# plurigrid/moose

Measured on AMD Instinct MI355X. Metric: replicated fixed(14,23) matmul elems/sec, higher is better.
Workload: dtype fixed(14,23) over Z_2^128 (exact multi-modular int8-MFMA GEMM)

## Files before the change

### csrc/gemm_crt.hip

```cpp
#include <hip/hip_runtime.h>

#include <algorithm>
#include <cmath>
#include <cstdint>
#include <cstdlib>
#include <cstring>
#include <mutex>

#include "hip_attr.h"
#include "moosex.h"

void mx_ws_note(int dev, int64_t want, bool ok);
bool mx_ws_malloc(void** p, int64_t bytes);
void mx_ws_shared_note(void);

namespace {

using u64 = uint64_t;
using u128 = unsigned __int128;
typedef int v4i __attribute__((ext_vector_type(4)));
typedef int v16i __attribute__((ext_vector_type(16)));

constexpr int kMaxMod = 48;
constexpr int kModuli[kMaxMod] = {256, 253, 251, 249, 247, 241, 239, 235, 233, 229, 227, 223,
                                  217, 211, 199, 197, 193, 191, 181, 179, 173, 167, 163, 157,
// ... 279 lines not shown
    emit(ob + boff);
    if (src.n > 0 && src.dual[b]) {
#pragma unroll
      for (int j = 0; j < 16; ++j) {
        const int64_t k = k0 + j;
        if (row < R && k < K) {
          T e = 0;
#pragma unroll
          for (int w = 0; w < NW; ++w) e |= (T)v[j][w] << (32 * w);
          e += TRANS ? x1[k * R + row] : x1[row * K + k];
#pragma unroll
          for (int w = 0; w < NW; ++w) v[j][w] = (uint32_t)(e >> (32 * w));
        }
      }
      emit(ob + src.dual[b] + boff);
    }
  }
}

template <class T>
__global__ void __launch_bounds__(256)
    k_add_pair(const T* __restrict__ a, const T* __restrict__ b, T* __restrict__ o, int64_t n) {
  for (int64_t i = blockIdx.x * (int64_t)blockDim.x + threadIdx.x; i < n;
       i += (int64_t)gridDim.x * blockDim.x)
    o[i] = a[i] + b[i];
}

__device__ inline int64_t xcd_remap(int64_t bid, int64_t nwg) {
  const int64_t q = nwg / 8, r = nwg % 8;
  const int64_t x = bid % 8;
// ... 691 lines not shown
      hipLaunchKernelGGL((k_crt_prep<T, true, 128, false>), grid, dim3(256), 0, st, X0, X1, R, K,
                         xs, mode, out, tiles, nkb, nkb_s, tb.pb, src);
    return;
  }
  if (!is_b)
    hipLaunchKernelGGL((k_crt_prep<T, false, BM>), grid, dim3(256), 0, st, X0, X1, R, K, xs, mode,
                       out, tiles, nkb, nkb_s, tb.pa, src);
  else if (rows == 256)
    hipLaunchKernelGGL((k_crt_prep<T, true, 256>), grid, dim3(256), 0, st, X0, X1, R, K, xs, mode,
                       out, tiles, nkb, nkb_s, tb.pb, src);
  else
    hipLaunchKernelGGL((k_crt_prep<T, true, 128>), grid, dim3(256), 0, st, X0, X1, R, K, xs, mode,
                       out, tiles, nkb, nkb_s, tb.pb, src);
}

int dma_mask() {
  const char* e = std::getenv("MOOSEX_CRT_DMA_MASK");
  return e ? std::atoi(e) : 3;
}

template <int WR, int WC, int BN, int MINW, bool M16, int STG = kStages, int IL = 0>
void launch_variant(const CPlan& p, const Tables& tb, int64_t batch, const int8_t* ra,
                    const int8_t* rb, int8_t* cr, int bcast, int roll, hipStream_t st,
                    int amap = 0, int bmap = 0) {
  constexpr int lds = STG * (kImg + BN * BK);
  const void* fn = M16 ? (const void*)k_crt_gemm16<WR, WC, BN, MINW, STG, IL>
                       : (const void*)k_crt_gemm<WR, WC, BN, MINW>;
  ensure_lds_attr(fn, lds, st);
  const dim3 grid((unsigned)(p.tiles_m * p.tiles_n), (unsigned)(batch * p.n));
  if constexpr (M16)
// ... 127 lines not shown
    rb = rbw;
  }
  if (roll)
    launch_prep<T>(p, tb, false, batch, M, K, a_bstride, A0, A0, 0, ra, st, p.a_nkb);
  else
    launch_prep<T>(p, tb, false, a_bc ? 1 : batch, M, K, a_bstride, A0, A1, mode, ra, st);
  launch_crt_gemm(p, tb, batch, ra, rb, cr, (a_bc ? 1 : 0) | (b_bc ? 2 : 0),
                  (int)(((roll % batch) + batch) % batch), st);
  launch_recon<T>(p, tb, batch, M, N, cr, C, accumulate, st);
  const hipError_t e = hipGetLastError();
  return e != hipSuccess ? -100 - (int)e : 0;
}

template <class T>
int run_crt_asym(int64_t M, int64_t N, int64_t K, const T* S0, const T* S1, const T* T0,
                 const T* T1, int rolled, T* C, hipStream_t st) {
  constexpr int words = sizeof(T) / 8;
  if (K % BK || !crt_mfma16()) return -7;
  if (2 * K > (1 << 15)) return -6;
  const CPlan p = make_cplan(words, 3, M, N, K, 1, true);
  if (p.n < 0) return -6;
  const Tables& tb = tables_for(words, p.n);
  const int64_t sa = M * K, sb = K * N;
  const T* a[3];
  const T* b[3];
  const T* c[3];
  const T* d[3];
  for (int q = 0; q < 3; ++q) {
    a[q] = S0 + q * sa;
    b[q] = rolled ? S0 + ((q + 1) % 3) * sa : S1 + q * sa;
    c[q] = T0 + q * sb;
// ... 15 lines not shown
    na = 5;
    nb = 5;
    amap = pmap(0, 1, 2, 3, 4);
    bmap = pmap(0, 1, 2, 3, 4);
  }
  const int64_t ra_bytes = na * a_entry, rb_bytes = nb * b_entry;
  static const bool asum = [] {
    const char* e = std::getenv("MOOSEX_CRT_ASUM");
    return !(e && e[0] == '0');
  }();
  static const bool dual = [] {
    const char* e = std::getenv("MOOSEX_CRT_DUAL");
    return !(e && e[0] == '0');
  }();
  const bool duals = rolled && dual;
  const int64_t sum_bytes = asum && !duals ? round_up(sa * (int64_t)sizeof(T), 256) : 0;
  int8_t* ws = (int8_t*)workspace(ra_bytes + rb_bytes + p.cr_bytes + sum_bytes, st);
  if (!ws) return -4;
  int8_t* ra = ws;
  int8_t* cr = ra + ra_bytes;
  int8_t* rb = cr + p.cr_bytes;
  T* a01 = sum_bytes ? (T*)(rb + rb_bytes) : nullptr;
  if (a01)
    hipLaunchKernelGGL((k_add_pair<T>), dim3((unsigned)std::min<int64_t>((sa + 255) / 256, 65536)),
                       dim3(256), 0, st, a[0], b[0], a01, sa);
  const int64_t kn = p.a_nkb;
  PrepSrcs sa_, sb_;
  auto put = [](PrepSrcs& q, const T* x0, const T* x1, int mode, int64_t dual = 0) {
    q.x0[q.n] = x0;
    q.x1[q.n] = x1;
    q.mode[q.n] = mode;
    q.dual[q.n] = dual;
    ++q.n;
  };
  if (duals) {
    put(sa_, a[2], a[2], 0);
    put(sa_, a[1], a[1], 0);
    put(sa_, a[0], b[0], 0, -3 * a_entry);
    put(sb_, d[1], c[1], 0, -b_entry);
    put(sb_, d[2], d[0], 0, -3 * b_entry);
    launch_prep<T>(p, tb, true, sb_.n, N, K, 0, nullptr, nullptr, 0, rb + 2 * b_entry, st, kn,
                   kn, sb_);
    launch_prep<T>(p, tb, false, sa_.n, M, K, 0, nullptr, nullptr, 0, ra + a_entry, st, kn, kn,
                   sa_);
  } else {
    if (a01)
      put(sa_, a01, a01, 0);
    else
      put(sa_, a[0], b[0], 2);
    put(sb_, c[0], d[0], 3);
    put(sb_, c[1], d[1], 3);
    if (rolled) {
      for (const T* e : {a[2], a[1], a[0]}) put(sa_, e, e, 0);
      for (const T* f : {d[1], d[2]}) put(sb_, f, f, 0);
    } else {
      for (const T* e : {b[1], a[1], a[2], b[2]}) put(sa_, e, e, 0);
      for (const T* f : {d[1], d[2], c[2]}) put(sb_, f, f, 0);
    }
    launch_prep<T>(p, tb, true, sb_.n, N, K, 0, nullptr, nullptr, 0, rb, st, kn, kn, sb_);
// ... 9 lines not shown

extern "C" {

int mx_gemm_asym(int words, int64_t M, int64_t N, int64_t K, const void* S0, const void* S1,
                 const void* T0, const void* T1, int rolled, void* C, void* stream) {
  if (M == 0 || N == 0) return 0;
  if (!rolled && (!S1 || !T1)) return -2;
  hipStream_t st = (hipStream_t)stream;
  if (words == 1)
    return run_crt_asym<u64>(M, N, K, (const u64*)S0, (const u64*)S1, (const u64*)T0,
                             (const u64*)T1, rolled, (u64*)C, st);
  if (words == 2)
    return run_crt_asym<u128>(M, N, K, (const u128*)S0, (const u128*)S1, (const u128*)T0,
                              (const u128*)T1, rolled, (u128*)C, st);
  return -2;
}

int mx_crt_moduli(int words, int64_t kprime) {
  if (words != 1 && words != 2) return -2;
  return moduli_needed(words, kprime);
}

int mx_crt_tables(int words, int n, int32_t* p_out, uint8_t* wa_out, uint8_t* wb_out,
                  int32_t* nega_out, int32_t* negb_out, uint16_t* W_out, uint16_t* Mw_out) {
  if ((words != 1 && words != 2) || n < 1 || n > kMaxMod) return -2;
  const Tables& t = tables_for(words, n);
  for (int i = 0; i < n; ++i) {
    p_out[i] = t.ep.p[i];
    for (int j = 0; j < 16; ++j) {
      wa_out[i * 16 + j] = (uint8_t)(t.pa.w[i][j / 4] >> (8 * (j % 4)));
// ... 108 lines not shown
```

### csrc/rss_fused.h

```cpp
#pragma once
#include <stdint.h>

#include "aes_core.h"
#include "ring_common.h"

namespace mxf {

template <class T>
MX_HD inline T shl(T x, int k) {
  constexpr int W = 8 * sizeof(T);
  return k >= W ? (T)0 : (T)(x << k);
}
template <class T>
MX_HD inline T shr(T x, int k) {
  constexpr int W = 8 * sizeof(T);
  return k >= W ? (T)0 : (T)(x >> k);
}

template <class T>
MX_HD inline T trunc_pr_z1(T x0, T x1, T x2, T r0, T r1, T rt0, T rm0, T z0, T z2, int m) {
  constexpr int W = 8 * sizeof(T);
  const int k = W - 1;
  T r = r0 + r1;
  T r_msb = shr<T>(r, W - 1);
  T r_top = shr<T>(shl<T>(r, 1), m + 1);
  T rt1 = r_top - rt0;
  T rm1 = r_msb - rm0;
  T mk0 = x0 + x1 + shl<T>((T)1, k - 1) + r0;
  T mk1 = x2 + r1;
  T c = mk0 + mk1;
  T c_msb = shr<T>(c, W - 1);
  T c_top = shr<T>(shl<T>(c, 1), m + 1);
  T ov0 = rm0 - shl<T>(c_msb * rm0, 1) + c_msb;
  T y0 = shl<T>(ov0, k - m) - rt0 + c_top - shl<T>((T)1, k - 1 - m);
  T ov1 = rm1 - shl<T>(c_msb * rm1, 1);
  T y1 = shl<T>(ov1, k - m) - rt1;
  return (y0 - z0) + (y1 - z2);
}

using u128_t = unsigned __int128;

constexpr int64_t kRingExtendLatMax = 8192;

MX_HD inline void ring_extend_dealer(uint64_t r0, uint64_t r1, u128_t R0, uint64_t M0, u128_t* R1,
                                     uint64_t* M1) {
  const uint64_t r = r0 + r1;
  *R1 = (u128_t)r - R0;
  *M1 = (r >> 63) - M0;
}

MX_HD inline uint64_t ring_extend_mask0(uint64_t x0, uint64_t x1, uint64_t r0) {
  return x0 + x1 + ((uint64_t)1 << 62) + r0;
// ... 99 lines not shown
```

### csrc/rss_fused.hip

```cpp
#include <hip/hip_runtime.h>

#include "prf_dev.h"
#include "moosex.h"
#include "ring_common.h"
#include "rss_fused.h"

using u64 = uint64_t;
using u128 = unsigned __int128;

namespace {

template <class T>
__global__ void __launch_bounds__(256) k_trunc_pr3(const T* __restrict__ s0, T* __restrict__ out0, T* __restrict__ out1,
                            int64_t n, int64_t os, T cm, int m, mxd::KeySrc keys, uint64_t n_r0, uint64_t n_r1,
                            uint64_t n_t, uint64_t n_m, uint64_t n_z0, uint64_t n_z2) {
  __shared__ uint32_t rks[2][mxd::kKeyWords];
  mxd::stage_keys(rks, keys, 2);
  constexpr int P = mxd::Lane<T>::kPer;
  const int64_t nb = (n + P - 1) / P;
  const uint32_t* const key[6] = {rks[0], rks[1], rks[0], rks[0], rks[0], rks[1]};
  const uint64_t nonce[6] = {n_r0, n_r1, n_t, n_m, n_z0, n_z2};
  mxd::walk_chunks<6>(nb, key, nonce, [&](int64_t b, const uint64_t (&lo)[6], const uint64_t (&hi)[6]) {
#pragma unroll
    for (int j = 0; j < P; ++j) {
// ... 202 lines not shown
          out1[os + i] = z2;
        }
        out1[2 * os + i] = a0;
      }
    }
    __syncthreads();
  }
}

template <class T>
__global__ void __launch_bounds__(256) k_share3(int kind, const void* __restrict__ xv, T* __restrict__ out0,
                         T* __restrict__ out1, int64_t n, int j0, mxd::KeySrc keys, uint64_t n1,
                         uint64_t na) {
  const bool mir = kind & MX_SHARE_MIRROR;
  kind &= ~MX_SHARE_MIRROR;
  const T* x = (const T*)xv;
  const double* xf = (const double*)xv;
  const double scale = kind == MX_SHARE_F64 ? ldexp(1.0, (int)na) : 0.0;
  __shared__ uint32_t rks[1][mxd::kKeyWords];
  mxd::stage_keys(rks, keys, 1);
  constexpr int P = mxd::Lane<T>::kPer;
  const int64_t nb = (n + P - 1) / P;
  const uint32_t* const key[1] = {rks[0]};
  const uint64_t nonce[1] = {n1};
  mxd::walk_chunks<1>(nb, key, nonce, [&](int64_t b, const uint64_t (&lo)[1], const uint64_t (&hi)[1]) {
#pragma unroll
    for (int j = 0; j < P; ++j) {
      const int64_t i = b * P + j;
      if (i >= n) break;
      const T r = mxd::pick<T>(lo[0], hi[0], j);
      const T xi = kind == MX_SHARE_F64 ? mxr::f64_to_ring<T>(xf[i] * scale) : x[i];
      const T v = kind == MX_CROSS_BOOL ? (T)(xi ^ r) : (T)(xi - r);
      T slot[3];
      slot[j0] = mir ? v : r;
      slot[(j0 + 1) % 3] = mir ? r : v;
      slot[(j0 + 2) % 3] = 0;
      const bool ring4 = out1 == out0 + n;
#pragma unroll
      for (int p = 0; p < 3; ++p) {
        out0[p * n + i] = slot[p];
        if (!ring4 || p == 2) out1[p * n + i] = slot[(p + 1) % 3];
      }
    }
  });
}

int launch_trunc_pr3(int words, const void* s0, void* out0, void* out1, int64_t n, int64_t os,
                     int m, const mxd::KeySrc& keys, const uint64_t* nn, void* stream,
                     const uint64_t* cm = nullptr) {
  const u64 c64 = cm ? cm[0] : 1;
  const u128 c128 = cm ? (((u128)cm[1] << 64) | cm[0]) : (u128)1;
// ... 160 lines not shown
```

### csrc/rss_fused_cpu.cpp

```cpp
#include <cmath>
#include <cstring>
#include <functional>
#include <vector>

#include "moosex.h"
#include "ring_common.h"
#include "rss_fused.h"

void mx_cpu_prf_range(const uint8_t* key, uint64_t nonce, int words, int64_t i0, int64_t n,
                      void* out);
void mx_cpu_parallel_for(int64_t n, int64_t grain,
                         const std::function<void(int64_t, int64_t)>& f);

extern "C" int mxh_trunc_pr3(int words, const void* s0, void* out0, void* out1, int64_t n, int m,
                             const uint8_t* k0, const uint8_t* k2, const uint64_t* nonces,
                             void* stream);
extern "C" int mxh_share3(int kind, int words, const void* x, void* out0, void* out1, int64_t n,
                          int j, const uint8_t* k_next, const uint8_t* k_all, uint64_t n1,
                          uint64_t na, void* stream);
extern "C" int mxh_trunc_pr3_k(int words, const void* s0, void* out0, void* out1, int64_t n,
                               int m, const uint32_t* slot_k0, const uint32_t* slot_k2,
                               const uint64_t* nonces, void* stream);
extern "C" int mxh_trunc_pr3_kmo(int words, const void* s0, void* out0, void* out1, int64_t n,
                                 int m, const uint32_t* slot_k0, const uint32_t* slot_k2,
// ... 103 lines not shown
          out[i] = (double)(int64_t)v * scale;
        else
          out[i] = mxr::i128_to_f64(v) * scale;
      }
    }
  });
  return 0;
}

template <class T>
int share3_host(int kind, const void* xv, T* out0, T* out1, int64_t n, int j, const uint8_t* kn,
                const uint8_t* , uint64_t n1, uint64_t na) {
  const bool mir = kind & MX_SHARE_MIRROR;
  kind &= ~MX_SHARE_MIRROR;
  const int words = sizeof(T) == 1 ? 0 : (int)(sizeof(T) / 8);
  const T* x = (const T*)xv;
  const double* xf = (const double*)xv;
  const double scale = kind == MX_SHARE_F64 ? std::ldexp(1.0, (int)na) : 0.0;
  mx_cpu_parallel_for(n, 1 << 12, [&](int64_t s, int64_t e) {
    const int64_t CH = 512;
    std::vector<T> r1(CH);
    for (int64_t c = s; c < e; c += CH) {
      int64_t len = std::min(CH, e - c);
      mx_cpu_prf_range(kn, n1, words, c, len, r1.data());
      for (int64_t t = 0; t < len; ++t) {
        int64_t i = c + t;
        const T xi = kind == MX_SHARE_F64 ? mxr::f64_to_ring<T>(xf[i] * scale) : x[i];
        const T v = kind == MX_CROSS_BOOL ? (T)(xi ^ r1[t]) : (T)(xi - r1[t]);
        T slot[3];
        slot[j] = mir ? v : r1[t];
        slot[(j + 1) % 3] = mir ? r1[t] : v;
        slot[(j + 2) % 3] = 0;
        for (int p = 0; p < 3; ++p) {
          out0[p * n + i] = slot[p];
          out1[p * n + i] = slot[(p + 1) % 3];
        }
      }
    }
  });
  return 0;
}

}

extern "C" {

int mx_trunc_pr3(int dev, int words, const void* s0, void* out0, void* out1, int64_t n, int m,
// ... 120 lines not shown
```

### moose_amd/ops/native.py

```python
from __future__ import annotations

import ctypes
import os
import threading

import torch

from moose_amd import errors
from moose_amd._native import build as _build

_LIB = None
_LOCK = threading.Lock()

c_i64 = ctypes.c_int64
c_int = ctypes.c_int
c_u64 = ctypes.c_uint64
c_vp = ctypes.c_void_p

_SIGS = {
    "mx_version": (c_int, []),
    "mx_device_count": (c_int, []),
    "mx_ew_binary": (c_int, [c_int, c_int, c_int, c_vp, c_i64, c_vp, c_i64, c_vp, c_i64, c_vp]),
    "mx_ew_unary": (c_int, [c_int, c_int, c_int, c_vp, c_vp, c_i64, c_i64, c_vp]),
    "mx_mul_add2": (c_int, [c_int, c_int, c_vp, c_vp, c_vp, c_vp, c_int, c_int, c_vp, c_vp,
# ... 224 lines not shown
                              c_vp, c_vp, c_vp, c_vp]),
    "mx_wsum_pair": (c_int, [c_int, c_int, c_int, c_int, c_int, c_int, c_int, c_i64, c_i64,
                             c_vp, c_vp, c_vp, c_vp, c_vp, c_vp, c_vp, c_vp, c_vp, c_vp, c_vp,
                             c_vp, c_vp, c_vp]),
    "mx_bits_b2a": (c_int, [c_int, c_int, c_int, c_int, c_i64, c_int, c_int, c_int, c_int,
                            c_vp, c_vp, c_vp,
                            c_vp, c_vp, c_vp, c_vp, c_vp, c_vp, c_vp, c_vp, c_vp]),
    "mx_key_refresh": (c_int, [c_vp, c_int, c_vp, c_vp, c_vp]),
    "mx_copy_async": (c_int, [c_vp, c_vp, ctypes.c_int64, c_vp]),
    "mx_key_refresh_host": (None, [c_vp, c_u64, c_int, c_vp]),
    "mx_copy_many": (c_int, [c_vp, c_int, c_i64, c_vp]),
    "mx_graph_free": (c_int, [c_vp, c_vp]),
    "mx_gemm_asym": (
        c_int, [c_int, c_i64, c_i64, c_i64, c_vp, c_vp, c_vp, c_vp, c_int, c_vp, c_vp],
    ),
    "mx_gemm_roll": (
        c_int,
        [c_int, c_i64, c_i64, c_i64, c_i64, c_vp, c_i64, c_i64, c_vp, c_vp, c_vp, c_vp, c_int,
         c_vp],
    ),
}


class NativeError(errors.KernelError):
    pass


def lib():
    global _LIB
    if _LIB is not None:
# ... 108 lines not shown
```

### moose_amd/ops/ring.py

```python
from __future__ import annotations

import builtins
import ctypes
import math
import os
import threading
from typing import List
from typing import Sequence

import numpy as np
import torch

from moose_amd.ops import native as nat

MASK64 = (1 << 64) - 1
MASK128 = (1 << 128) - 1

_BIN = {"add": 0, "sub": 1, "mul": 2, "and": 3, "or": 4, "xor": 5}
_UN = {"neg": 0, "not": 1, "shl": 2, "shr": 3, "sar": 4}
_CMP = {"lt": 0, "gt": 1, "eq": 2, "msb": 3}


_UPLOAD_HOOK = None
_TLS = threading.local()
# ... 952 lines not shown
            ts[1] = ts[3] = None
        if all(t is None or t.is_contiguous() for t in ts):
            out = empty((3, M, N), bits, d.device)
            rc = nat.lib().mx_gemm_asym(
                _words(bits), M, N, K, nat.ptr(ts[0]), None if ts[1] is None else nat.ptr(ts[1]),
                nat.ptr(ts[2]), None if ts[3] is None else nat.ptr(ts[3]), 1 if rolled else 0,
                nat.ptr(out.data), nat.stream_of(d))
            if rc != -7:
                nat.check(rc, "gemm_asym")
                return out
    if x1 is None or y1 is None:
        x1 = RT(torch.roll(x0.data, -1, dims=0), bits)
        y1 = RT(torch.roll(y0.data, -1, dims=0), bits)
    A0, A1, B0, B1 = _asym_operands(x0, x1, y0, y1)
    return dot_cross(A0, A1, B0, B1, nb=1)


def _party_batch_strides(t: RT):
    d = t.data
    el = 2 if t.bits == 128 else 1
    if d.dim() < 3:
        return None
    expect = 1
    for size, st in zip(reversed(d.shape[2:]), reversed(d.stride()[2:])):
        if size != 1 and st != expect:
            return None
        expect *= size
    if d.stride(0) % el or d.stride(1) % el:
        return None
    return d.stride(0) // el, d.stride(1) // el
# ... 1280 lines not shown
```

### moose_amd/protocols/fixedpoint.py

```python
from __future__ import annotations

import math
import os
from dataclasses import dataclass
from functools import lru_cache

import numpy as np
import torch

from moose_amd.ops import ring as R
from moose_amd.protocols import replicated as rep
from moose_amd.protocols.replicated import RepTensor
from moose_amd.runtime.session import PV
from moose_amd.runtime.values import MV


@dataclass
class RepFixed:
    t: RepTensor
    frac: int
    integ: int

    @property
    def bits(self):
# ... 182 lines not shown
    return _with(xs[0], t) if isinstance(xs[0], RepFixed) else t


def broadcast_to(sess, x, shape):
    if tuple(shape_of(sess, x)) == tuple(shape):
        return x
    return local(sess, x, "Broadcast", shape=tuple(shape))


def shape_of(sess, x):
    t = x.t if isinstance(x, RepFixed) else x
    if isinstance(t, MV):
        return tuple(t.v.shape)
    if isinstance(t, rep.PendingTrunc) and not t.completed:
        return sess.p_shape(PV(t.plc, t.v_add))
    return sess.p_shape(t.s0)


def static_shape(sess, x):
    try:
        return shape_of(sess, x)
    except ValueError:
        return None


def broadcast_like(sess, small: RepTensor, big: RepTensor) -> RepTensor:
    shape = static_shape(sess, big)
    if shape is not None:
        return rep.local(sess, small, "Broadcast", shape=tuple(shape))
    s0, s1 = rep._sharewise(sess, "BroadcastLike", small.plc, (small.s0, small.s1),
# ... 924 lines not shown
```

### moose_amd/protocols/replicated.py

```python
from __future__ import annotations

import os
from dataclasses import dataclass
from typing import Optional

import torch

from moose_amd.ir.computation import ReplicatedPlacement
from moose_amd.ops import ring as R
from moose_amd.runtime.session import HV
from moose_amd.runtime.session import PV
from moose_amd.runtime.session import Public
from moose_amd.utils.telemetry import span


@dataclass
class RepTensor:
    plc: ReplicatedPlacement
    bits: int
    kind: str
    s0: PV
    s1: PV
    zero_slot: Optional[int] = None

# ... 167 lines not shown

    @s0.setter
    def s0(self, v):
        self._s0 = v

    @property
    def s1(self):
        self.finish()
        return self._s1

    @s1.setter
    def s1(self, v):
        self._s1 = v


def lazy(x) -> bool:
    return ((isinstance(x, PendingTrunc) and (not x.completed or x._rb is not None))
            or isinstance(x, DeferredRep) or (isinstance(x, StackedTail) and not x.done))


def settle(x):
    if isinstance(x, PendingTrunc):
        x._complete()
    elif isinstance(x, DeferredRep):
        x._tail.finish()
    elif isinstance(x, StackedTail):
        x.finish()


def _reveal_pending(sess, x: PendingTrunc, host):
    from moose_amd.parallel.spmd import Remote

    plc = x.plc
    if host not in plc.owners or getattr(sess, "party_dot_trunc", None) is None \
            or not hasattr(sess, "party_exchange") or getattr(sess, "is_simulated", True):
        return None
    j = plc.owners.index(host)
    idx = sess.party_index(plc)
    nonces = tuple(sess.nonce(plc) for _ in range(7))
    x.completed = True
    if idx is None:
# ... 25 lines not shown


def share(sess, plc, x: HV, kind="arith") -> RepTensor:
    bits = x.v.bits if hasattr(x.v, "bits") else None
    with span("rep.share"):
        sess.setup(plc)
        shape = sess.h("Shape", x.host, x)
        j = _owner_index(plc, x.host)
        if j is None:
            return _share_outsider(sess, plc, x, kind, bits, shape)
        sub = "Sub" if kind == "arith" else "Xor"
        o = plc.owners
        j1, j2 = (j + 1) % 3, (j + 2) % 3
        n1, na = sess.nonce(plc), sess.nonce(plc)
        if getattr(sess, "fused", False):
            s0, s1 = sess.fused_share(plc, x, j, kind, n1, na)
            return RepTensor(plc, bits, kind, s0, s1, zero_slot=j2)
        party = getattr(sess, "party_share", None)
        if party is not None and bits in (64, 128):
            s0, s1 = party(plc, x, j, kind, n1, na)
            return RepTensor(plc, bits, kind, s0, s1, zero_slot=j2)
        d = sess.share_dir(plc, j) if hasattr(sess, "share_dir") else 1
        zero = lambda h: sess.h("Fill", o[h], shape, value=0, bits=bits)
        if d == 1:
            r_j = sess.h_prf(plc, o[j], j, shape, bits, n1)
            r_j2 = sess.h_prf(plc, o[j2], j, shape, bits, n1)
            xj1 = sess.h(sub, o[j], x, r_j)
            comp0 = {j: r_j, j1: sess.move(xj1, o[j1]), j2: zero(j2)}
            comp1 = {j: xj1, j1: zero(j1), j2: r_j2}
        else:
# ... 383 lines not shown
        return None
    terms = [_cross_terms(p, x.zero_slot, y.zero_slot) for p in range(3)]
    if any(t is None or t[0] == "zero" for t in terms):
        return None
    bits = x.bits

    def pick(name, s0, s1, p):
        a, b = R.RT(s0.data[p], bits), R.RT(s1.data[p], bits)
        return a if name[1:] == "0" else b if name[1:] == "1" else R.binary("add", a, b)

    A = torch.stack([pick(a, xs0, xs1, p).data for p, (a, _) in enumerate(terms)])
    B = torch.stack([pick(b, ys0, ys1, p).data for p, (_, b) in enumerate(terms)])
    return PV(x.plc, R.dot(R.RT(A, bits), R.RT(B, bits), nb=1))


def dot(sess, x: RepTensor, y: RepTensor, nbatch: int = 0) -> RepTensor:
    with span("rep.dot"):
        over = getattr(sess, "p_dot_zs_reshare", None)
        if over is not None and getattr(sess, "fused", False) and not nbatch:
            res = over(x.plc, x.s0, x.s1, y.s0, y.s1, x.kind)
            if res is not None:
                return RepTensor(x.plc, x.bits, x.kind, res[0], res[1])
        if nbatch:
            v = sess.p_dot_cross(x.plc, x.s0, x.s1, y.s0, y.s1, nbatch=nbatch)
        else:
            v = _zero_slot_cross(sess, x, y) or sess.p_dot_cross(x.plc, x.s0, x.s1, y.s0,
                                                                    y.s1)
        fused = getattr(sess, "p_zero_share_reshare", None)
        if fused is not None and getattr(sess, "fused", False):
            s0, s1 = fused(x.plc, v, x.kind)
# ... 21 lines not shown
            return RepTensor(x.plc, x.bits, "arith", s0, s1)
    if chunks > 1:
        xs, ys = x.s0.v.shape, y.s0.v.shape
        if len(xs) == 3 and len(ys) == 3:
            M = xs[1]
            nchunk = min(chunks, M // 128)
    party = getattr(sess, "party_dot_trunc", None)
    use_party = (party is not None and m and 0 < m <= 63 and x.kind == "arith"
                 and x.bits in (64, 128) and os.environ.get("MOOSEX_DOT_TAIL", "1") != "0")
    if nchunk <= 1:
        tail = getattr(sess, "p_zs_trunc", None)
        if (tail is not None and m and x.kind == "arith" and getattr(sess, "fused", False)
                and getattr(sess, "device", None) is not None and sess.device.type == "cuda"
                and os.environ.get("MOOSEX_DOT_TAIL", "1") != "0"):
            with span("rep.dot_trunc_fused"):
                v = _zero_slot_cross(sess, x, y) or sess.p_dot_cross(x.plc, x.s0, x.s1, y.s0,
                                                                        y.s1)
                issue = getattr(sess, "p_zs_trunc_issue", None)
                if (issue is not None and x.bits in (64, 128)
                        and os.environ.get("MOOSEX_DOT_OPEN", "1") != "0"):
                    return StackedTail(sess, x.plc, x.bits, v, m, issue(x.plc, v))
                s0, s1 = tail(x.plc, v, m)
                return RepTensor(x.plc, x.bits, "arith", s0, s1)
        if use_party:
            with span("rep.dot_trunc_party"):
                nonces = tuple(sess.nonce(x.plc) for _ in range(7))
                pre_fn = getattr(sess, "party_dot_trunc_pre", None)
                pre = pre_fn(x.plc, x, y, m, nonces) if pre_fn is not None else None
                v = _zero_slot_cross(sess, x, y) or sess.p_dot_cross(x.plc, x.s0, x.s1, y.s0,
                                                                        y.s1)
                if getattr(sess, "defer_reshare", False) and pre is not None:
                    s0, s1, rb = party(x.plc, v, m, nonces, pre=pre, defer=True)
# ... 356 lines not shown
```

### moose_amd/runtime/session.py

```python
from __future__ import annotations

import math
import os
import threading
from contextlib import contextmanager
from dataclasses import dataclass
from typing import Any
from typing import List
from typing import Optional

import numpy as np
import torch

from moose_amd.ir.computation import ReplicatedPlacement
from moose_amd.ops import ring as R
from moose_amd.runtime import lanes as _lanes
from moose_amd.runtime.prims import PRIMS
from moose_amd.utils import telemetry


@dataclass
class HV:
    host: str
    v: Any
# ... 834 lines not shown
            ctypes.c_void_p(self.key_ptr(plc, 0)), ctypes.c_void_p(self.key_ptr(plc, 2)), nn, ca,
            nat.stream_of(d)), "wsum_trunc3")
        x = type("X", (), {})()
        x.plc = plc
        self._trunc_traffic(x, out0.numel() * out0.element_size() // 3)
        return PV(plc, R.RT(out0, v.bits)), PV(plc, R.RT(out1, v.bits))

    def _trunc_traffic(self, x, nbytes):
        o = x.plc.owners
        st = self.stats
        for src, dst in ((o[2], o[1]), (o[0], o[1]), (o[1], o[0])):
            st.record_send(src, dst, nbytes, count=2)
        st.record_round(2 * nbytes, count=2)

    def fused_share(self, plc, x: HV, j, kind, n1, na):
        import ctypes

        from moose_amd.ops import native as nat

        code, xd, aux = R.share_source(x.v, kind)
        d = self.share_dir(plc, j)
        out0, out1 = (t.data for t in R.ring4((3,) + tuple(x.v.shape), x.v.bits, xd.device))
        nat.check(
            nat.lib().mx_share3_k(
                nat.dev_of(xd), code | (R.SHARE_MIRROR if d == 2 else 0), R._words(x.v.bits),
                nat.ptr(xd), nat.ptr(out0), nat.ptr(out1), x.v.numel(), j,
                ctypes.c_void_p(self.key_ptr(plc, (j + d - 1) % 3)),
                ctypes.c_void_p(self.key_ptr(plc, 3)), n1, na if aux is None else aux,
                nat.stream_of(xd),
            ),
            "share3",
        )
        self.stats.record_send(x.host, plc.owners[(j + d) % 3], _nbytes(x.v))
        return PV(plc, R.RT(out0, x.v.bits)), PV(plc, R.RT(out1, x.v.bits))

    def mirror(self, x: HV, plc):
        from moose_amd.runtime.values import MV

        for o in plc.owners:
            if o != x.host:
                self.stats.record_send(x.host, o, _nbytes(x.v))
        return MV(plc, x.v)

    def materialized(self, x) -> bool:
        return True


def _stack3(v):
    if isinstance(v, R.RT):
# ... 3 lines not shown
```

Baseline: 1.400 billion.

## Fuse input secret-sharing PRF into CRT GEMM operand prep via lazy shares

Adds a LazyShare tensor that defers materializing replicated shares of a freshly shared input. When such a share feeds a replicated dot, a new prep kernel regenerates the ChaCha mask and masked value on the fly and writes CRT residue images straight into the GEMM operand buffers. This skips writing and re-reading the three share planes in memory and drops the separate share3 kernel launch. In exchange, the prep kernel does extra PRF work per tile and adds a narrow fast path with many shape and mode conditions.

New measurement: 1.432 billion, median of 6. +2.2%, better.

```diff
diff --git a/csrc/gemm_crt.hip b/csrc/gemm_crt.hip
--- a/csrc/gemm_crt.hip
+++ b/csrc/gemm_crt.hip
@@ -9,6 +9,8 @@
 
 #include "hip_attr.h"
 #include "moosex.h"
+#include "prf_dev.h"
+#include "rss_fused.h"
 
 void mx_ws_note(int dev, int64_t want, bool ok);
 bool mx_ws_malloc(void** p, int64_t bytes);
@@ -318,6 +320,144 @@
         }
       }
       emit(ob + src.dual[b] + boff);
+    }
+  }
+}
+
+struct ShareSrc {
+  const void* x = nullptr;
+  int kind = 0;
+  int frac = 0;
+  int j0 = 0;
+  uint64_t nonce = 0;
+  mxd::KeySrc key;
+};
+struct SrcPlan {
+  const void* x;
+  int kind, pad;
+  double scale;
+  uint64_t nonce;
+  int ph[4];
+  int64_t off[4];
+};
+
+template <bool TRANS, int ROWS, bool PK>
+__global__ void __launch_bounds__(256)
+    k_crt_prep_src(const SrcPlan s, const mxd::KeySrc keys, int64_t R, int64_t K,
+                   int8_t* __restrict__ out, int64_t tiles, int64_t nkb, const PrepTab tab) {
+  using T = u128;
+  constexpr int NW = 4;
+  __shared__ uint32_t rks[1][mxd::kKeyWords];
+  __shared__ uint4 xch[4][4][64];
+  mxd::stage_keys(rks, keys, 1);
+  const int lane = threadIdx.x & 63;
+  const int p = lane & 3;
+  uint4(*xw)[64] = xch[threadIdx.x >> 6];
+  const int n = tab.n;
+  const int64_t plane = tiles * nkb * (int64_t)(ROWS * BK);
+  const int64_t total = tiles * ROWS * nkb * 4;
+  for (int64_t g = blockIdx.x * (int64_t)blockDim.x + threadIdx.x; g < total;
+       g += (int64_t)gridDim.x * blockDim.x) {
+    const int c = (int)((g >> 2) & 3);
+    const int rlow = (int)((g >> 4) & 3);
+    const int64_t rest = g >> 6;
+    int64_t row, kb, i0, istep;
+    if (!TRANS) {
+      const int64_t q = rest / (ROWS / 4);
+      kb = 4 * (q % (nkb / 4)) + p;
+      row = (q / (nkb / 4)) * ROWS + (rest % (ROWS / 4)) * 4 + rlow;
+      i0 = row * K + (kb - p) * BK + c * 16;
+      istep = 1;
+    } else {
+      const int64_t q = rest >> 4;
+      kb = q % nkb;
+      row = (q / nkb) * 256 + 64 * p + (rest & 15) * 4 + rlow;
+      i0 = (kb * BK + c * 16) * R + (row - 64 * p);
+      istep = R;
+    }
+    const bool live = row < R;
+    const int64_t t = row / ROWS;
+    const int r = (int)(row % ROWS);
+    uint32_t v[16][NW];
+#pragma unroll
+    for (int jj = 0; jj < 4; ++jj) {
+      uint32_t w[16];
+      mx::chacha_block(rks[0], s.nonce, mx::ks_block_of((uint64_t)(i0 + (4 * jj + p) * istep)), w);
+#pragma unroll
+      for (int q = 0; q < 4; ++q)
+        xw[q][lane ^ q] = make_uint4(w[4 * q], w[4 * q + 1], w[4 * q + 2], w[4 * q + 3]);
+      __builtin_amdgcn_fence(__ATOMIC_RELEASE, "wavefront");
+      __builtin_amdgcn_wave_barrier();
+      __builtin_amdgcn_fence(__ATOMIC_ACQUIRE, "wavefront");
+#pragma unroll
+      for (int u = 0; u < 4; ++u) {
+        const uint4 e = xw[p][((lane & ~3) | u) ^ p];
+        v[4 * jj + u][0] = live ? e.x : 0u;
+        v[4 * jj + u][1] = live ? e.y : 0u;
+        v[4 * jj + u][2] = live ? e.z : 0u;
+        v[4 * jj + u][3] = live ? e.w : 0u;
+      }
+      __builtin_amdgcn_fence(__ATOMIC_RELEASE, "wavefront");
+      __builtin_amdgcn_wave_barrier();
+      __builtin_amdgcn_fence(__ATOMIC_ACQUIRE, "wavefront");
+    }
+    const int64_t boff = (t * nkb + kb) * (int64_t)(ROWS * BK) + img_off(r, c);
+    auto emit = [&](int8_t* base) __attribute__((always_inline)) {
+      {
+        int rr[16];
+#pragma unroll
+        for (int j = 0; j < 16; ++j) rr[j] = (int)(v[j][0] * tab.mul0);
+        v4i o;
+#pragma unroll
+        for (int u = 0; u < 4; ++u) o[u] = (int)pack4(rr[4 * u], rr[4 * u + 1], rr[4 * u + 2], rr[4 * u + 3]);
+        *(v4i*)base = o;
+      }
+      for (int i = 1; i < n; ++i) {
+        const uint32_t w[4] = {tab.w[i][0], tab.w[i][1], tab.w[i][2], tab.w[i][3]};
+        const uint32_t neg = tab.neg[i];
+        const float pf = (float)tab.p[i], rcp = tab.rcp[i];
+        int rr[16];
+        if constexpr (PK) {
+#pragma unroll
+          for (int j = 0; j < 16; j += 2)
+            residue2<NW>(v[j], v[j + 1], w, neg, pf, rcp, rr[j], rr[j + 1]);
+        } else {
+#pragma unroll
+          for (int j = 0; j < 16; ++j) rr[j] = residue<NW>(v[j], w, neg, pf, rcp);
+        }
+        v4i o;
+#pragma unroll
+        for (int u = 0; u < 4; ++u) o[u] = (int)pack4(rr[4 * u], rr[4 * u + 1], rr[4 * u + 2], rr[4 * u + 3]);
+        *(v4i*)(base + i * plane) = o;
+      }
+    };
+    auto step = [&](bool sum) __attribute__((always_inline)) {
+#pragma unroll
+      for (int j = 0; j < 16; ++j) {
+        T h = 0;
+#pragma unroll
+        for (int w = 0; w < NW; ++w) h |= (T)v[j][w] << (32 * w);
+        const T x = live ? mxf::share_plain<T>(s.kind, s.x, i0 + 64 * p + j * istep, s.scale) : (T)0;
+        const T other = mxf::share_masked<T>(s.kind, x, h);
+        h = sum ? (T)(h + other) : other;
+#pragma unroll
+        for (int w = 0; w < NW; ++w) v[j][w] = (uint32_t)(h >> (32 * w));
+      }
+    };
+#pragma nounroll
+    for (int ph = 0; ph < 4; ++ph) {
+      if (s.ph[0] != ph && s.ph[1] != ph && s.ph[2] != ph && s.ph[3] != ph) continue;
+      if (ph == 1) step(false);
+      if (ph == 2) step(true);
+      if (ph == 3) {
+#pragma unroll
+        for (int j = 0; j < 16; ++j)
+#pragma unroll
+          for (int w = 0; w < NW; ++w) v[j][w] = 0;
+      }
+#pragma nounroll
+      for (int e = 0; e < 4; ++e)
+        if (s.ph[e] == ph) emit(out + s.off[e] + boff);
     }
   }
 }
@@ -1039,6 +1179,45 @@
                        out, tiles, nkb, nkb_s, tb.pb, src);
 }
 
+bool share_src_ok(const ShareSrc& s) {
+  const int kind = s.kind & ~MX_SHARE_MIRROR;
+  return s.x && (kind == MX_CROSS_ARITH || kind == MX_SHARE_F64) && s.j0 >= 0 && s.j0 < 3;
+}
+
+void launch_prep_src(const CPlan& p, const Tables& tb, bool is_b, const ShareSrc& src, int64_t R,
+                     int64_t K, int8_t* out, int64_t entry, hipStream_t st) {
+  static const int kSlotsA[4][2] = {{0, 1}, {2, -1}, {1, -1}, {0, -1}};
+  static const int kSlotsB[4][2] = {{0, 1}, {1, 2}, {2, -1}, {0, -1}};
+  const int kind = src.kind & ~MX_SHARE_MIRROR;
+  int jr, jv;
+  mxf::share_place(src.j0, (src.kind & MX_SHARE_MIRROR) != 0, &jr, &jv);
+  SrcPlan s;
+  s.x = src.x;
+  s.kind = kind;
+  s.pad = 0;
+  s.scale = kind == MX_SHARE_F64 ? std::ldexp(1.0, src.frac) : 0.0;
+  s.nonce = src.nonce;
+  for (int e = 0; e < 4; ++e) {
+    const int* sl = is_b ? kSlotsB[e] : kSlotsA[e];
+    const bool has_r = sl[0] == jr || sl[1] == jr, has_v = sl[0] == jv || sl[1] == jv;
+    s.ph[e] = has_r && has_v ? 2 : has_r ? 0 : has_v ? 1 : 3;
+    s.off[e] = e * entry;
+  }
+  const int64_t tiles = is_b ? p.tiles_n : p.tiles_m;
+  const int rows = is_b ? p.bn : BM;
+  const int64_t work = tiles * rows * p.a_nkb * 4;
+  const dim3 grid((unsigned)std::min<int64_t>(work / 256, 16384));
+  if (!is_b)
+    hipLaunchKernelGGL((k_crt_prep_src<false, BM, true>), grid, dim3(256), 0, st, s, src.key, R, K,
+                       out, tiles, p.a_nkb, tb.pa);
+  else if (rows == 256)
+    hipLaunchKernelGGL((k_crt_prep_src<true, 256, false>), grid, dim3(256), 0, st, s, src.key, R,
+                       K, out, tiles, p.a_nkb, tb.pb);
+  else
+    hipLaunchKernelGGL((k_crt_prep_src<true, 128, false>), grid, dim3(256), 0, st, s, src.key, R,
+                       K, out, tiles, p.a_nkb, tb.pb);
+}
+
 int dma_mask() {
   const char* e = std::getenv("MOOSEX_CRT_DMA_MASK");
   return e ? std::atoi(e) : 3;
@@ -1196,7 +1375,8 @@
 
 template <class T>
 int run_crt_asym(int64_t M, int64_t N, int64_t K, const T* S0, const T* S1, const T* T0,
-                 const T* T1, int rolled, T* C, hipStream_t st) {
+                 const T* T1, int rolled, T* C, hipStream_t st, const ShareSrc* xs = nullptr,
+                 const ShareSrc* ys = nullptr) {
   constexpr int words = sizeof(T) / 8;
   if (K % BK || !crt_mfma16()) return -7;
   if (2 * K > (1 << 15)) return -6;
@@ -1242,6 +1422,11 @@
     return !(e && e[0] == '0');
   }();
   const bool duals = rolled && dual;
+  if (xs || ys) {
+    if (words != 2 || !duals) return -7;
+    if (xs && (K % 256 || !share_src_ok(*xs))) return -7;
+    if (ys && (N % 256 || !share_src_ok(*ys))) return -7;
+  }
   const int64_t sum_bytes = asum && !duals ? round_up(sa * (int64_t)sizeof(T), 256) : 0;
   int8_t* ws = (int8_t*)workspace(ra_bytes + rb_bytes + p.cr_bytes + sum_bytes, st);
   if (!ws) return -4;
@@ -1267,10 +1452,16 @@
     put(sa_, a[0], b[0], 0, -3 * a_entry);
     put(sb_, d[1], c[1], 0, -b_entry);
     put(sb_, d[2], d[0], 0, -3 * b_entry);
-    launch_prep<T>(p, tb, true, sb_.n, N, K, 0, nullptr, nullptr, 0, rb + 2 * b_entry, st, kn,
-                   kn, sb_);
-    launch_prep<T>(p, tb, false, sa_.n, M, K, 0, nullptr, nullptr, 0, ra + a_entry, st, kn, kn,
-                   sa_);
+    if (ys)
+      launch_prep_src(p, tb, true, *ys, N, K, rb, b_entry, st);
+    else
+      launch_prep<T>(p, tb, true, sb_.n, N, K, 0, nullptr, nullptr, 0, rb + 2 * b_entry, st, kn,
+                     kn, sb_);
+    if (xs)
+      launch_prep_src(p, tb, false, *xs, M, K, ra, a_entry, st);
+    else
+      launch_prep<T>(p, tb, false, sa_.n, M, K, 0, nullptr, nullptr, 0, ra + a_entry, st, kn, kn,
+                     sa_);
   } else {
     if (a01)
       put(sa_, a01, a01, 0);
@@ -1310,6 +1501,29 @@
     return run_crt_asym<u128>(M, N, K, (const u128*)S0, (const u128*)S1, (const u128*)T0,
                               (const u128*)T1, rolled, (u128*)C, st);
   return -2;
+}
+
+int mx_gemm_asym_src(int words, int64_t M, int64_t N, int64_t K, const void* S0, const void* T0,
+                     const int64_t* xsrc, const int64_t* ysrc, void* C, void* stream) {
+  if (M == 0 || N == 0) return 0;
+  if (words != 2) return -7;
+  if ((!xsrc && !S0) || (!ysrc && !T0)) return -2;
+  ShareSrc sx, sy;
+  auto fill = [](ShareSrc& s, const int64_t* a) {
+    s.x = (const void*)(intptr_t)a[0];
+    s.kind = (int)a[1];
+    s.frac = (int)a[2];
+    s.j0 = (int)a[3];
+    const uint32_t* slot[1] = {(const uint32_t*)(intptr_t)a[4]};
+    s.key = mxd::keysrc_slots(slot, 1);
+    s.nonce = (uint64_t)a[5];
+  };
+  if (xsrc) fill(sx, xsrc);
+  if (ysrc) fill(sy, ysrc);
+  if ((xsrc && !sx.key.slot[0]) || (ysrc && !sy.key.slot[0])) return -2;
+  return run_crt_asym<u128>(M, N, K, (const u128*)S0, nullptr, (const u128*)T0, nullptr, 1,
+                            (u128*)C, (hipStream_t)stream, xsrc ? &sx : nullptr,
+                            ysrc ? &sy : nullptr);
 }
 
 int mx_crt_moduli(int words, int64_t kprime) {
diff --git a/csrc/rss_fused.h b/csrc/rss_fused.h
--- a/csrc/rss_fused.h
+++ b/csrc/rss_fused.h
@@ -2,6 +2,7 @@
 #include <stdint.h>
 
 #include "aes_core.h"
+#include "moosex.h"
 #include "ring_common.h"
 
 namespace mxf {
@@ -36,6 +37,27 @@
   T ov1 = rm1 - shl<T>(c_msb * rm1, 1);
   T y1 = shl<T>(ov1, k - m) - rt1;
   return (y0 - z0) + (y1 - z2);
+}
+
+template <class T>
+MX_HD inline T share_plain(int kind, const void* xv, int64_t i, double scale) {
+  return kind == MX_SHARE_F64 ? mxr::f64_to_ring<T>(((const double*)xv)[i] * scale)
+                              : ((const T*)xv)[i];
+}
+template <class T>
+MX_HD inline T share_masked(int kind, T x, T r) {
+  return kind == MX_CROSS_BOOL ? (T)(x ^ r) : (T)(x - r);
+}
+MX_HD inline void share_place(int j0, bool mir, int* jr, int* jv) {
+  *jr = mir ? (j0 + 1) % 3 : j0;
+  *jv = mir ? j0 : (j0 + 1) % 3;
+}
+template <class T>
+MX_HD inline void share_slots(int kind, T x, T r, int j0, bool mir, T (&slot)[3]) {
+  const T v = share_masked<T>(kind, x, r);
+  slot[j0] = mir ? v : r;
+  slot[(j0 + 1) % 3] = mir ? r : v;
+  slot[(j0 + 2) % 3] = 0;
 }
 
 using u128_t = unsigned __int128;
diff --git a/csrc/rss_fused.hip b/csrc/rss_fused.hip
--- a/csrc/rss_fused.hip
+++ b/csrc/rss_fused.hip
@@ -240,8 +240,6 @@
                          uint64_t na) {
   const bool mir = kind & MX_SHARE_MIRROR;
   kind &= ~MX_SHARE_MIRROR;
-  const T* x = (const T*)xv;
-  const double* xf = (const double*)xv;
   const double scale = kind == MX_SHARE_F64 ? ldexp(1.0, (int)na) : 0.0;
   __shared__ uint32_t rks[1][mxd::kKeyWords];
   mxd::stage_keys(rks, keys, 1);
@@ -255,12 +253,8 @@
       const int64_t i = b * P + j;
       if (i >= n) break;
       const T r = mxd::pick<T>(lo[0], hi[0], j);
-      const T xi = kind == MX_SHARE_F64 ? mxr::f64_to_ring<T>(xf[i] * scale) : x[i];
-      const T v = kind == MX_CROSS_BOOL ? (T)(xi ^ r) : (T)(xi - r);
       T slot[3];
-      slot[j0] = mir ? v : r;
-      slot[(j0 + 1) % 3] = mir ? r : v;
-      slot[(j0 + 2) % 3] = 0;
+      mxf::share_slots<T>(kind, mxf::share_plain<T>(kind, xv, i, scale), r, j0, mir, slot);
       const bool ring4 = out1 == out0 + n;
 #pragma unroll
       for (int p = 0; p < 3; ++p) {
diff --git a/csrc/rss_fused_cpu.cpp b/csrc/rss_fused_cpu.cpp
--- a/csrc/rss_fused_cpu.cpp
+++ b/csrc/rss_fused_cpu.cpp
@@ -141,8 +141,6 @@
   const bool mir = kind & MX_SHARE_MIRROR;
   kind &= ~MX_SHARE_MIRROR;
   const int words = sizeof(T) == 1 ? 0 : (int)(sizeof(T) / 8);
-  const T* x = (const T*)xv;
-  const double* xf = (const double*)xv;
   const double scale = kind == MX_SHARE_F64 ? std::ldexp(1.0, (int)na) : 0.0;
   mx_cpu_parallel_for(n, 1 << 12, [&](int64_t s, int64_t e) {
     const int64_t CH = 512;
@@ -152,12 +150,8 @@
       mx_cpu_prf_range(kn, n1, words, c, len, r1.data());
       for (int64_t t = 0; t < len; ++t) {
         int64_t i = c + t;
-        const T xi = kind == MX_SHARE_F64 ? mxr::f64_to_ring<T>(xf[i] * scale) : x[i];
-        const T v = kind == MX_CROSS_BOOL ? (T)(xi ^ r1[t]) : (T)(xi - r1[t]);
         T slot[3];
-        slot[j] = mir ? v : r1[t];
-        slot[(j + 1) % 3] = mir ? r1[t] : v;
-        slot[(j + 2) % 3] = 0;
+        mxf::share_slots<T>(kind, mxf::share_plain<T>(kind, xv, i, scale), r1[t], j, mir, slot);
         for (int p = 0; p < 3; ++p) {
           out0[p * n + i] = slot[p];
           out1[p * n + i] = slot[(p + 1) % 3];
diff --git a/moose_amd/ops/native.py b/moose_amd/ops/native.py
--- a/moose_amd/ops/native.py
+++ b/moose_amd/ops/native.py
@@ -262,6 +262,9 @@
     "mx_gemm_asym": (
         c_int, [c_int, c_i64, c_i64, c_i64, c_vp, c_vp, c_vp, c_vp, c_int, c_vp, c_vp],
     ),
+    "mx_gemm_asym_src": (
+        c_int, [c_int, c_i64, c_i64, c_i64, c_vp, c_vp, c_vp, c_vp, c_vp, c_vp],
+    ),
     "mx_gemm_roll": (
         c_int,
         [c_int, c_i64, c_i64, c_i64, c_i64, c_vp, c_i64, c_i64, c_vp, c_vp, c_vp, c_vp, c_int,
diff --git a/moose_amd/ops/ring.py b/moose_amd/ops/ring.py
--- a/moose_amd/ops/ring.py
+++ b/moose_amd/ops/ring.py
@@ -990,6 +990,35 @@
         y1 = RT(torch.roll(y0.data, -1, dims=0), bits)
     A0, A1, B0, B1 = _asym_operands(x0, x1, y0, y1)
     return dot_cross(A0, A1, B0, B1, nb=1)
+
+
+def dot_cross_asym_src(x0, y0, xsrc, ysrc, M: int, K: int, N: int):
+    ts = [None if t is None else t.data for t in (x0, y0)]
+    if any(t is not None and not t.is_contiguous() for t in ts):
+        return None
+    words = []
+    for s in (xsrc, ysrc):
+        if s is None:
+            words.append(None)
+            continue
+        code, d, frac, j0, slot, nonce = s
+        if not d.is_cuda or not d.is_contiguous():
+            return None
+        words.append((ctypes.c_int64 * 6)(d.data_ptr(), code, int(frac or 0), j0, int(slot),
+                                          _i64(nonce)))
+    anyt = next(s[1] for s in (xsrc, ysrc) if s is not None)
+    out = empty((3, M, N), 128, anyt.device)
+    rc = nat.lib().mx_gemm_asym_src(2, M, N, K, nat.ptr(ts[0]), nat.ptr(ts[1]), words[0],
+                                    words[1], nat.ptr(out.data), nat.stream_of(anyt))
+    if rc == -7:
+        return None
+    nat.check(rc, "gemm_asym_src")
+    return out
+
+
+def _i64(v: int) -> int:
+    v &= (1 << 64) - 1
+    return v - (1 << 64) if v >> 63 else v
 
 
 def _party_batch_strides(t: RT):
diff --git a/moose_amd/protocols/fixedpoint.py b/moose_amd/protocols/fixedpoint.py
--- a/moose_amd/protocols/fixedpoint.py
+++ b/moose_amd/protocols/fixedpoint.py
@@ -220,6 +220,8 @@
         return tuple(t.v.shape)
     if isinstance(t, rep.PendingTrunc) and not t.completed:
         return sess.p_shape(PV(t.plc, t.v_add))
+    if isinstance(t, rep.LazyShare) and not t.done:
+        return t.shape
     return sess.p_shape(t.s0)
 
 
diff --git a/moose_amd/protocols/replicated.py b/moose_amd/protocols/replicated.py
--- a/moose_amd/protocols/replicated.py
+++ b/moose_amd/protocols/replicated.py
@@ -205,9 +205,53 @@
         self._s1 = v
 
 
+class LazyShare(RepTensor):
+
+    def __init__(self, sess, plc, bits, kind, issued, zero_slot):
+        self._sess, self._issued = sess, issued
+        self._stream = R._stream_of(issued[1])
+        super().__init__(plc, bits, kind, None, None, zero_slot=zero_slot)
+
+    @property
+    def done(self) -> bool:
+        return self._s0 is not None
+
+    @property
+    def shape(self):
+        return tuple(self._issued[6])
+
+    def source(self):
+        return None if self.done else self._issued
+
+    def finish(self):
+        if self._s0 is None:
+            R._join(self._stream)
+            self._s0, self._s1 = self._sess.fused_share_run(self.plc, self._issued)
+            self._issued = None
+
+    @property
+    def s0(self):
+        self.finish()
+        return self._s0
+
+    @s0.setter
+    def s0(self, v):
+        self._s0 = v
+
+    @property
+    def s1(self):
+        self.finish()
+        return self._s1
+
+    @s1.setter
+    def s1(self, v):
+        self._s1 = v
+
+
 def lazy(x) -> bool:
     return ((isinstance(x, PendingTrunc) and (not x.completed or x._rb is not None))
-            or isinstance(x, DeferredRep) or (isinstance(x, StackedTail) and not x.done))
+            or isinstance(x, DeferredRep)
+            or (isinstance(x, (StackedTail, LazyShare)) and not x.done))
 
 
 def settle(x):
@@ -215,7 +259,7 @@
         x._complete()
     elif isinstance(x, DeferredRep):
         x._tail.finish()
-    elif isinstance(x, StackedTail):
+    elif isinstance(x, (StackedTail, LazyShare)):
         x.finish()
 
 
@@ -271,6 +315,10 @@
         j1, j2 = (j + 1) % 3, (j + 2) % 3
         n1, na = sess.nonce(plc), sess.nonce(plc)
         if getattr(sess, "fused", False):
+            prep = getattr(sess, "share_prep", None)
+            if prep is not None and prep(x, kind):
+                return LazyShare(sess, plc, bits, kind,
+                                 sess.fused_share_issue(plc, x, j, kind, n1, na), j2)
             s0, s1 = sess.fused_share(plc, x, j, kind, n1, na)
             return RepTensor(plc, bits, kind, s0, s1, zero_slot=j2)
         party = getattr(sess, "party_share", None)
@@ -684,6 +732,13 @@
     return PV(x.plc, R.dot(R.RT(A, bits), R.RT(B, bits), nb=1))
 
 
+def _dot_cross_src(sess, x: RepTensor, y: RepTensor):
+    if not any(isinstance(t, LazyShare) and not t.done for t in (x, y)):
+        return None
+    fn = getattr(sess, "p_dot_cross_src", None)
+    return fn(x.plc, x, y) if fn is not None else None
+
+
 def dot(sess, x: RepTensor, y: RepTensor, nbatch: int = 0) -> RepTensor:
     with span("rep.dot"):
         over = getattr(sess, "p_dot_zs_reshare", None)
@@ -735,8 +790,8 @@
                 and getattr(sess, "device", None) is not None and sess.device.type == "cuda"
                 and os.environ.get("MOOSEX_DOT_TAIL", "1") != "0"):
             with span("rep.dot_trunc_fused"):
-                v = _zero_slot_cross(sess, x, y) or sess.p_dot_cross(x.plc, x.s0, x.s1, y.s0,
-                                                                        y.s1)
+                v = (_zero_slot_cross(sess, x, y) or _dot_cross_src(sess, x, y)
+                     or sess.p_dot_cross(x.plc, x.s0, x.s1, y.s0, y.s1))
                 issue = getattr(sess, "p_zs_trunc_issue", None)
                 if (issue is not None and x.bits in (64, 128)
                         and os.environ.get("MOOSEX_DOT_OPEN", "1") != "0"):
diff --git a/moose_amd/runtime/session.py b/moose_amd/runtime/session.py
--- a/moose_amd/runtime/session.py
+++ b/moose_amd/runtime/session.py
@@ -872,25 +872,58 @@
         st.record_round(2 * nbytes, count=2)
 
     def fused_share(self, plc, x: HV, j, kind, n1, na):
-        import ctypes
-
-        from moose_amd.ops import native as nat
-
+        return self.fused_share_run(plc, self.fused_share_issue(plc, x, j, kind, n1, na))
+
+    def share_prep(self, x: HV, kind) -> bool:
+        return (self.device.type == "cuda" and kind == "arith" and x.v.bits == 128
+                and len(x.v.shape) == 2 and self.pair_rolled and self.dot_asym
+                and not _lanes.ACTIVE
+                and os.environ.get("MOOSEX_SHARE_PREP", "1") != "0")
+
+    def fused_share_issue(self, plc, x: HV, j, kind, n1, na):
         code, xd, aux = R.share_source(x.v, kind)
         d = self.share_dir(plc, j)
-        out0, out1 = (t.data for t in R.ring4((3,) + tuple(x.v.shape), x.v.bits, xd.device))
+        self.stats.record_send(x.host, plc.owners[(j + d) % 3], _nbytes(x.v))
+        return (code | (R.SHARE_MIRROR if d == 2 else 0), xd, na if aux is None else aux, j,
+                self.key_ptr(plc, (j + d - 1) % 3), n1, tuple(x.v.shape), x.v.bits)
+
+    def fused_share_run(self, plc, issued):
+        import ctypes
+
+        from moose_amd.ops import native as nat
+
+        code, xd, na, j, slot, n1, shape, bits = issued
+        out0, out1 = (t.data for t in R.ring4((3,) + shape, bits, xd.device))
         nat.check(
             nat.lib().mx_share3_k(
-                nat.dev_of(xd), code | (R.SHARE_MIRROR if d == 2 else 0), R._words(x.v.bits),
-                nat.ptr(xd), nat.ptr(out0), nat.ptr(out1), x.v.numel(), j,
-                ctypes.c_void_p(self.key_ptr(plc, (j + d - 1) % 3)),
-                ctypes.c_void_p(self.key_ptr(plc, 3)), n1, na if aux is None else aux,
-                nat.stream_of(xd),
+                nat.dev_of(xd), code, R._words(bits), nat.ptr(xd), nat.ptr(out0), nat.ptr(out1),
+                math.prod(shape), j, ctypes.c_void_p(slot),
+                ctypes.c_void_p(self.key_ptr(plc, 3)), n1, na, nat.stream_of(xd),
             ),
             "share3",
         )
-        self.stats.record_send(x.host, plc.owners[(j + d) % 3], _nbytes(x.v))
-        return PV(plc, R.RT(out0, x.v.bits)), PV(plc, R.RT(out1, x.v.bits))
+        return PV(plc, R.RT(out0, bits)), PV(plc, R.RT(out1, bits))
+
+    def p_dot_cross_src(self, plc, x, y):
+        srcs = [t.source() if hasattr(t, "source") else None for t in (x, y)]
+        if (srcs[0] is None and srcs[1] is None) or x.bits != 128 or _lanes.ACTIVE:
+            return None
+        shp = [tuple(s[6]) if s is not None else tuple(t.s0.v.shape[1:])
+               for s, t in zip(srcs, (x, y))]
+        if len(shp[0]) != 2 or len(shp[1]) != 2 or shp[0][1] != shp[1][0]:
+            return None
+        (M, K), (_, N) = shp
+        if min(M, K, N) < 256:
+            return None
+        stacks = [None if s is not None else t.s0.v for s, t in zip(srcs, (x, y))]
+        if not all(s is None or isinstance(s, R.RT) for s in stacks):
+            return None
+        for s, t in zip(srcs, (x, y)):
+            if s is not None:
+                R._join(t._stream)
+        out = R.dot_cross_asym_src(stacks[0], stacks[1],
+                                   *[None if s is None else s[:6] for s in srcs], M, K, N)
+        return None if out is None else PV(plc, out)
 
     def mirror(self, x: HV, plc):
         from moose_amd.runtime.values import MV
```
